# jcatalang/LUDVM

Hardware: AMD Instinct MI355X
Metric: biot_savart_pair_interactions_per_s (higher is better)
Workload: dtype f32

## Files before the change

ludvm_amd/csrc/pair_sym_kernels.hpp:

```cpp
#pragma once
#include <hip/hip_runtime.h>
#include "pair_kernels.hpp"
#include "sym_rule.hpp"

namespace ludvm {

struct SymScale {
  float scale;
  float pad;
  double inv;
};

struct SymArgs {
  const float* x; const float* z; const float* g;
  const float* xl; const float* zl;
  const float* cx; const float* cz;
  long long n;
  long long ntiles;
  long long dmax;
  long long i_first;
  long long i_count;
  int ysplit;
  int rsplit;
  int ytail;
  int rbulk;
  int xcd_run;
  long long tail_items;
  int diag_only;
  int tune_split, tune_rsplit;
  long long* acc_u; long long* acc_w;
  const SymScale* scale;
  long long* bad;
  float vc4;
  const long long* n_dev;
  int shard_rank, shard_world;
};

__device__ __forceinline__ unsigned long long fx_units(float v, float scale) {
  const float t = v * scale;
  const float a = __builtin_fabsf(t);
  const float h = __builtin_floorf(a * 2.3283064365386963e-10f);
  const float r = __builtin_fmaf(-h, 4294967296.0f, a);
  const unsigned long long m = ((unsigned long long)(unsigned)h << 32) | (unsigned long long)(unsigned)r;
  const unsigned long long s = (unsigned long long)((long long)__builtin_bit_cast(int, t) >> 31);
  return (m ^ s) - s;
}
__device__ __forceinline__ void fx_add(long long* acc, float v, float scale) {
  atomicAdd(reinterpret_cast<unsigned long long*>(acc), fx_units(v, scale));
}

__device__ __forceinline__ float dpp_rol1(float v) {
  const int i = __builtin_bit_cast(int, v);
  return __builtin_bit_cast(float, __builtin_amdgcn_update_dpp(i, i, 0x134, 0xf, 0xf, false));
}
__device__ __forceinline__ f32x2 dpp_rol1(f32x2 v) { return (f32x2){dpp_rol1(v.x), dpp_rol1(v.y)}; }

__device__ __forceinline__ f32x2 pk_sub_sel(f32x2 p, f32x2 s, int half) {
  f32x2 d;
  if (half) asm("v_pk_add_f32 %0, %1, %2 op_sel:[1,0] op_sel_hi:[1,1] neg_lo:[0,1] neg_hi:[0,1]" : "=v"(d) : "v"(p), "v"(s));
  else asm("v_pk_add_f32 %0, %1, %2 op_sel:[0,0] op_sel_hi:[0,1] neg_lo:[0,1] neg_hi:[0,1]" : "=v"(d) : "v"(p), "v"(s));
  return d;
}
__device__ __forceinline__ f32x2 pk_mul_sel(f32x2 s, f32x2 p, int half, f32x2 after) {
  f32x2 d;
  if (half) asm("v_pk_mul_f32 %0, %1, %2 op_sel:[0,1] op_sel_hi:[1,1]" : "=v"(d) : "v"(s), "v"(p), "v"(after));
  else asm("v_pk_mul_f32 %0, %1, %2 op_sel:[0,0] op_sel_hi:[1,0]" : "=v"(d) : "v"(s), "v"(p), "v"(after));
  return d;
}

__device__ __forceinline__ float load_or(const float* p, unsigned i, unsigned n, float pad) {
  const float v = p[i < n ? i : 0u];
  return i < n ? v : pad;
}

constexpr int kPlane = 96 * 4;
template <int T, int PLANE = kPlane>
__device__ __forceinline__ void slab_store(float* l, int home4, const float (&v)[T]) {
#pragma unroll
  for (int q = 0; q < T / 4; ++q) {
    const f32x4 V = (f32x4){v[4 * q], v[4 * q + 1], v[4 * q + 2], v[4 * q + 3]};
    *reinterpret_cast<f32x4*>(&l[q * PLANE + home4]) = V;
    if (PLANE > 256 && home4 < 128) *reinterpret_cast<f32x4*>(&l[q * PLANE + 256 + home4]) = V;
  }
}
template <int T, int PLANE = kPlane>
__device__ __forceinline__ void slab_load(const float* l, int home4, f32x2 (&out)[T / 2]) {
#pragma unroll
  for (int q = 0; q < T / 4; ++q) {
    const f32x4 V = *reinterpret_cast<const f32x4*>(&l[q * PLANE + home4]);
    out[2 * q] = (f32x2){V.x, V.y};
    out[2 * q + 1] = (f32x2){V.z, V.w};
  }
}

template <int T, bool HILO = false, int R = 1, bool RED = (R != 1)>
__global__ void __launch_bounds__(kBlock) __attribute__((amdgpu_waves_per_eu(T == 8 || HILO ? 3 : 4)))
pair_sym_f32(SymArgs a) {
  static_assert(T == 4 || T == 8, "T vortices per lane, read as T/4 ds_read_b128 per component");
  static_assert(R == 0 || R == 1 || R == 2 || R == 4, "waves per item");
  static_assert(RED == (R != 1), "one wave per item has nothing to reduce");
  constexpr int RR = R == 0 ? 4 : R;
  unsigned n = (unsigned)a.n, ntiles = (unsigned)a.ntiles, dmax = (unsigned)a.dmax, i_first = (unsigned)a.i_first,
           i_count = (unsigned)a.i_count;
  int ysplit = a.diag_only ? 1 : a.ysplit, ytail = a.ytail, rbulk = a.rbulk;
  if (a.n_dev) {
    n = (unsigned)*a.n_dev;
    unsigned dtot_;
    int rs_;
    sym_geometry_t<unsigned>(n, T, a.tune_split, R == 0 ? -1 : R, (unsigned)a.tail_items, ntiles, dmax, dtot_, ysplit, rs_, ytail,
                             rbulk);
    i_first = 0;
    i_count = ntiles;
    if (a.shard_world > 1) {
      unsigned long long f, cnt;
      shard_block(ntiles, a.shard_rank, a.shard_world, &f, &cnt);
      i_first = (unsigned)f;
      i_count = (unsigned)cnt;
    }
    if (a.diag_only) ysplit = 1;
  }
  constexpr int H = T / 2;
  constexpr int kWaves = kBlock / 64;
  constexpr int kComp = HILO ? 5 : 3;
  __shared__ __attribute__((aligned(16))) float slab[kWaves][kComp][(T / 4) * kPlane];
  static_assert(2 * T * 64 <= kComp * (T / 4) * kPlane, "partial sums fit the slab");
  __shared__ __attribute__((aligned(16))) float ioff[HILO ? 1 : kWaves][HILO ? 1 : 2][HILO ? 4 : 64 * T];

  const int lane = threadIdx.x & 63;
  const int wv = __builtin_amdgcn_readfirstlane((int)(threadIdx.x >> 6));
  const unsigned xcd = blockIdx.x % (unsigned)kXcds, qb = blockIdx.x / (unsigned)kXcds;
  unsigned yq = 0, unit = 0;
  bool active, shared;
  int rr = RR;
  if constexpr (R == 0) {
    const unsigned y1 = (unsigned)(ysplit - ytail);
    const unsigned rb = (unsigned)rbulk, ipb = (unsigned)kWaves / rb;
    const unsigned n_bulk = (unsigned)xcd_items(i_count, (unsigned)ysplit, xcd, 0, y1, a.xcd_run);
    const unsigned nb1 = (n_bulk * rb + 3) / 4;
    const bool tail = qb >= nb1;
    rr = tail ? 4 : (int)rb;
    shared = rr > 1;
    const unsigned q = tail ? qb - nb1 : qb * ipb + (unsigned)wv / rb;
    active = tail ? xcd_item(i_count, (unsigned)ysplit, xcd, y1, (unsigned)ytail, q, yq, unit, a.xcd_run)
                  : (q < n_bulk && xcd_item(i_count, (unsigned)ysplit, xcd, 0, y1, q, yq, unit, a.xcd_run));
    const bool wg_active = tail ? active : qb * ipb < n_bulk;
    if (!wg_active || (!shared && !active)) return;
  } else {
    shared = R > 1;
    const unsigned q = qb * (kWaves / R) + wv / R;
    active = xcd_item(i_count, (unsigned)ysplit, xcd, 0, (unsigned)ysplit, q, yq, unit, a.xcd_run);
  }
  const int r = shared ? wv % rr : 0;
  const int w0 = wv - r;
  if (R == 1 && !active) return;
  if (!active) { yq = 0; unit = 0; }
  const unsigned I = i_first + unit;
  const int y = (int)yq;
  const int ksteps = shared ? 64 / rr : 64;
  const int k_lo = r * ksteps;
  const int k_hi = k_lo + ksteps;
  constexpr unsigned W = 64u * T;
  float* const lx = slab[wv][0];
  float* const lz = slab[wv][1];
  float* const lg = slab[wv][2];
  float* const lxl = slab[wv][HILO ? 3 : 0];
  float* const lzl = slab[wv][HILO ? 4 : 1];

  const bool even = (ntiles % 2 == 0) && ntiles > 1;
  const int dtot = (int)dmax + (even ? 1 : 0);
  const int per = a.diag_only ? 0 : (int)(((unsigned)dtot + (unsigned)ysplit - 1) / (unsigned)ysplit);
  const int d_lo = 1 + y * per;
  int d_hi = d_lo + per;
  if (d_hi > dtot + 1) d_hi = dtot + 1;

  constexpr int NS = T / 4;
  f32x2 xp[H], zp[H], gp[H], au[T], aw[T], xpl[H], zpl[H];
  f32x2 xq[2][H], zq[2][H];
  {
    float x0[T], z0[T], g0[T], xl0[T], zl0[T];
#pragma unroll
    for (int t = 0; t < T; ++t) {
      const unsigned i = I * W + lane + 64u * t;
      const unsigned nl = active ? n : 0u;
      x0[t] = load_or(a.x, i, nl, kPadPosF); z0[t] = load_or(a.z, i, nl, kPadPosF); g0[t] = load_or(a.g, i, nl, 0.0f);
      xl0[t] = HILO ? load_or(a.xl, i, nl, 0.0f) : 0.0f; zl0[t] = HILO ? load_or(a.zl, i, nl, 0.0f) : 0.0f;
      au[t] = (f32x2){0.f, 0.f}; aw[t] = (f32x2){0.f, 0.f};
    }
#pragma unroll
    for (int h = 0; h < H; ++h) {
      xp[h] = (f32x2){x0[2 * h], x0[2 * h + 1]}; zp[h] = (f32x2){z0[2 * h], z0[2 * h + 1]};
      gp[h] = (f32x2){g0[2 * h], g0[2 * h + 1]};
      xpl[h] = (f32x2){xl0[2 * h], xl0[2 * h + 1]}; zpl[h] = (f32x2){zl0[2 * h], zl0[2 * h + 1]};
      xq[0][h] = xp[h]; xq[1][h] = xp[h]; zq[0][h] = zp[h]; zq[1][h] = zp[h];
    }
    if constexpr (!HILO) { slab_store<T, 256>(ioff[wv][0], lane * 4, x0); slab_store<T, 256>(ioff[wv][1], lane * 4, z0); }
  }
  const f32x2 vc4 = {a.vc4, a.vc4};
  const float fxs = a.scale->scale;
  const bool local = !HILO && a.cx != nullptr;
  const bool pl = (lane & 1) != 0;
  struct Org { float x0, x1, z0, z1; };
  auto scalar = [](float v) { return __builtin_bit_cast(float, __builtin_amdgcn_readfirstlane(__builtin_bit_cast(int, v))); };
  auto origin_records = [&](unsigned b) -> Org {
    const bool has = local && (b << kOriginShift) < n;
    const unsigned s0 = has ? 2 * b : 0;
    Org o{0.0f, 0.0f, 0.0f, 0.0f};
    if (has) { o.x0 = a.cx[s0]; o.x1 = a.cx[s0 + 1]; o.z0 = a.cz[s0]; o.z1 = a.cz[s0 + 1]; }
    return o;
  };
  auto to_scalars = [&](const Org& v) -> Org { return Org{scalar(v.x0), scalar(v.x1), scalar(v.z0), scalar(v.z1)}; };
  const unsigned blk_i = (I * W) >> kOriginShift;
  Org oi[NS];
#pragma unroll
  for (int q = 0; q < NS; ++q) oi[q] = to_scalars(origin_records(blk_i + q));
  float oix[NS], oiz[NS];
#pragma unroll
  for (int q = 0; q < NS; ++q) { oix[q] = pl ? oi[q].x1 : oi[q].x0; oiz[q] = pl ? oi[q].z1 : oi[q].z0; }
  auto refer_targets = [&](const Org oj) {
    f32x2 xo[H], zo[H];
    slab_load<T, 256>(ioff[HILO ? 0 : wv][0], lane * 4, xo);
    slab_load<T, 256>(ioff[HILO ? 0 : wv][HILO ? 0 : 1], lane * 4, zo);
#pragma unroll
    for (int rr = 0; rr < 2; ++rr) {
      const bool odd = pl != (rr != 0);
      const float jx = odd ? oj.x1 : oj.x0, jz = odd ? oj.z1 : oj.z0;
#pragma unroll
      for (int h = 0; h < H; ++h) {
        const float ddx = oix[h / 2] - jx, ddz = oiz[h / 2] - jz;
        xq[rr][h] = xo[h] + (f32x2){ddx, ddx};
        zq[rr][h] = zo[h] + (f32x2){ddz, ddz};
      }
    }
  };
  auto load_plane = [&](const float* l, int q, int pos4, f32x2 (&out)[2]) {
    const f32x4 V = *reinterpret_cast<const f32x4*>(&l[q * kPlane + pos4]);
    out[0] = (f32x2){V.x, V.y};
    out[1] = (f32x2){V.z, V.w};
  };
  float chk = 0.0f;
  const int lane32x4 = ((lane + 32) & 63) * 4;

  struct Round { unsigned J; bool diag, valid; };
  auto round_of = [&](int dd) -> Round {
    Round rd;
    rd.diag = dd < 0;
    const int d = rd.diag ? 0 : d_lo + dd;
    rd.valid = rd.diag || (active && dd < per && d < d_hi && !(even && d == dtot && I >= ntiles / 2));
    rd.J = I + (unsigned)d;
    if (rd.J >= ntiles) rd.J -= ntiles;
    return rd;
  };
  float pjx[T], pjz[T], pjg[T], pjxl[T], pjzl[T];
  Org poj[NS];
  auto fetch_tile = [&](const Round& rd) {
    const unsigned Jt = rd.valid ? rd.J : I;
    if ((Jt + 1) * W <= n) {
#pragma unroll
      for (int t = 0; t < T; ++t) {
        const unsigned j = Jt * W + lane + 64u * t;
        pjx[t] = a.x[j]; pjz[t] = a.z[j]; pjg[t] = a.g[j];
        pjxl[t] = HILO ? a.xl[j] : 0.0f; pjzl[t] = HILO ? a.zl[j] : 0.0f;
      }
    } else {
#pragma unroll
      for (int t = 0; t < T; ++t) {
        const unsigned j = Jt * W + lane + 64u * t;
        pjx[t] = load_or(a.x, j, n, kPadPosF); pjz[t] = load_or(a.z, j, n, kPadPosF); pjg[t] = load_or(a.g, j, n, 0.0f);
        pjxl[t] = HILO ? load_or(a.xl, j, n, 0.0f) : 0.0f; pjzl[t] = HILO ? load_or(a.zl, j, n, 0.0f) : 0.0f;
      }
    }
#pragma unroll
    for (int q = 0; q < NS; ++q) poj[q] = origin_records(((Jt * W) >> kOriginShift) + q);
  };
  constexpr bool kPrefetch = R != 0;
  const int dd0 = (active && y == 0) ? -1 : 0;
  if (kPrefetch) fetch_tile(round_of(dd0));
  for (int dd = dd0; dd < per; ++dd) {
    const Round rd = round_of(dd);
    if (!kPrefetch) fetch_tile(rd);
    const bool diag = rd.diag, valid = rd.valid;
    const unsigned J = rd.J;
    f32x2 bu[H], bw[H];
#pragma unroll
    for (int m = 0; m < H; ++m) { bu[m] = (f32x2){0.f, 0.f}; bw[m] = (f32x2){0.f, 0.f}; }
    Org oj[NS];
#pragma unroll
    for (int q = 0; q < NS; ++q) oj[q] = to_scalars(poj[q]);
    if (valid) {
      slab_store<T>(lx, lane * 4, pjx); slab_store<T>(lz, lane * 4, pjz); slab_store<T>(lg, lane * 4, pjg);
      if (HILO) { slab_store<T>(lxl, lane * 4, pjxl); slab_store<T>(lzl, lane * 4, pjzl); }
      __builtin_amdgcn_fence(__ATOMIC_RELEASE, "wavefront");
      __builtin_amdgcn_wave_barrier();
      __builtin_amdgcn_fence(__ATOMIC_ACQUIRE, "wavefront");
    }
    if (kPrefetch && dd + 1 < per) fetch_tile(round_of(dd + 1));
    if (valid) {

#pragma unroll
      for (int q = 0; q < NS; ++q) {
        if (local) refer_targets(oj[q]);
        for (int k = k_lo; k < k_hi; k += 2) {
          const int pos0 = ((k & 32) ? lane32x4 : lane * 4) + (k & 31) * 4;
#pragma unroll
          for (int rr = 0; rr < 2; ++rr) {
            const int pos = pos0 + 4 * rr;
            f32x2 xj[2], zj[2], gj[2], xjl[2], zjl[2];
            load_plane(lx, q, pos, xj); load_plane(lz, q, pos, zj); load_plane(lg, q, pos, gj);
            if (HILO) { load_plane(lxl, q, pos, xjl); load_plane(lzl, q, pos, zjl); }
#pragma unroll
            for (int mm = 0; mm < 2; ++mm) {
              const int m = 2 * q + mm;
#pragma unroll
              for (int t = 0; t < T; ++t) {
                f32x2 dx = pk_sub_sel(HILO ? xp[t / 2] : xq[rr][t / 2], xj[mm], t & 1);
                f32x2 dz = pk_sub_sel(HILO ? zp[t / 2] : zq[rr][t / 2], zj[mm], t & 1);
                if (HILO) { dx = dx + pk_sub_sel(xpl[t / 2], xjl[mm], t & 1); dz = dz + pk_sub_sel(zpl[t / 2], zjl[mm], t & 1); }
                f32x2 r2 = dx * dx;
                r2 = __builtin_elementwise_fma(dz, dz, r2);
                const f32x2 qq = __builtin_elementwise_fma(r2, r2, vc4);
                const f32x2 sv = {__builtin_amdgcn_rsqf(qq.x), __builtin_amdgcn_rsqf(qq.y)};
                const f32x2 sj = sv * gj[mm];
                const f32x2 si = pk_mul_sel(sv, gp[t / 2], t & 1, sj);
                au[t] = __builtin_elementwise_fma(dz, sj, au[t]);
                aw[t] = __builtin_elementwise_fma(dx, sj, aw[t]);
                bu[m] = __builtin_elementwise_fma(dz, si, bu[m]);
                bw[m] = __builtin_elementwise_fma(dx, si, bw[m]);
              }
            }
#pragma unroll
            for (int mm = 0; mm < 2; ++mm) { bu[2 * q + mm] = dpp_rol1(bu[2 * q + mm]); bw[2 * q + mm] = dpp_rol1(bw[2 * q + mm]); }
          }
        }
      }
      __builtin_amdgcn_fence(__ATOMIC_RELEASE, "wavefront");
      __builtin_amdgcn_wave_barrier();
    }
    const int home = (lane + k_hi) & 63;
    if (diag) continue;
    if (!RED || !shared) {
      if (valid) {
#pragma unroll
        for (int m = 0; m < H; ++m) {
          const unsigned j0 = J * W + home + 64u * (2 * m), j1 = j0 + 64;
          if (j0 < n) { fx_add(&a.acc_u[j0], -bu[m].x, fxs); fx_add(&a.acc_w[j0], -bw[m].x, fxs); }
          if (j1 < n) { fx_add(&a.acc_u[j1], -bu[m].y, fxs); fx_add(&a.acc_w[j1], -bw[m].y, fxs); }
        }
      }
    } else {
      if (valid) {
#pragma unroll
        for (int m = 0; m < H; ++m) {
          lx[(4 * m + 0) * 64 + home] = bu[m].x; lx[(4 * m + 1) * 64 + home] = bu[m].y;
          lx[(4 * m + 2) * 64 + home] = bw[m].x; lx[(4 * m + 3) * 64 + home] = bw[m].y;
        }
      }
      __syncthreads();
      if (valid) {
#pragma unroll 1
        for (int c = r; c < 2 * T; c += rr) {
          float v = 0.0f;
#pragma unroll
          for (int q = 0; q < RR; ++q)
            if (R != 0 || q < rr) v += (&slab[w0 + q][0][0])[c * 64 + lane];
          const unsigned j = J * W + lane + 64u * (2 * (c / 4) + (c & 1));
          if (j < n) fx_add((c & 2) ? &a.acc_w[j] : &a.acc_u[j], -v, fxs);
        }
      }
      __syncthreads();
    }
  }

  if (!RED || !shared) {
#pragma unroll
    for (int t = 0; t < T; ++t) {
      const unsigned i = I * W + lane + 64u * t;
      if (i < n) {
        const float su = au[t].x + au[t].y, sw = aw[t].x + aw[t].y;
        fx_add(&a.acc_u[i], su, fxs); fx_add(&a.acc_w[i], sw, fxs);
        chk += su + sw;
      }
    }
  } else {
#pragma unroll
    for (int t = 0; t < T; ++t) { lx[(2 * t) * 64 + lane] = au[t].x + au[t].y; lx[(2 * t + 1) * 64 + lane] = aw[t].x + aw[t].y; }
    __syncthreads();
    if (active) {
#pragma unroll 1
      for (int c = r; c < 2 * T; c += rr) {
        float v = 0.0f;
#pragma unroll
        for (int q = 0; q < RR; ++q)
          if (R != 0 || q < rr) v += (&slab[w0 + q][0][0])[c * 64 + lane];
        const unsigned i = I * W + lane + 64u * (c / 2);
        if (i < n) { fx_add((c & 1) ? &a.acc_w[i] : &a.acc_u[i], v, fxs); chk += v; }
      }
    }
  }
  if (!(__builtin_fabsf(chk) < __builtin_inff())) atomicAdd(reinterpret_cast<unsigned long long*>(a.bad), 1ULL);
}

template <int T>
__global__ void __launch_bounds__(kBlock) __attribute__((amdgpu_waves_per_eu(3)))
pair_sym_quad_f32(SymArgs a) {
  static_assert(T == 8, "the quad variant is built for the 512-vortex tile");
  constexpr int H = T / 2, NS = T / 4;
  constexpr unsigned W = 64u * T;
  constexpr int kWaves = kBlock / 64;
  static_assert(kWaves == (int)kQuad, "one I tile per wave");
  __shared__ __attribute__((aligned(16))) float slab[3][(T / 4) * kPlane];
  __shared__ __attribute__((aligned(16))) float ex[kWaves][2 * T * 64];
  __shared__ __attribute__((aligned(16))) float ioff[kWaves][2][64 * T];

  unsigned n = (unsigned)a.n, i_first = (unsigned)a.i_first, i_count = (unsigned)a.i_count;
  if (a.n_dev) {
    n = (unsigned)*a.n_dev;
    const unsigned nt = (n + W - 1) / W;
    i_first = 0;
    i_count = nt;
    if (a.shard_world > 1) {
      unsigned long long f, cnt;
      shard_block(nt, a.shard_rank, a.shard_world, &f, &cnt);
      i_first = (unsigned)f;
      i_count = (unsigned)cnt;
    }
  }
  const QuadGeom gm = quad_geometry<unsigned>(n, T, a.tune_split);
  const unsigned ntiles = gm.ntiles, dmax = gm.dmax;
  const int dtot = (int)gm.dtot;
  const bool even = (ntiles % 2 == 0) && ntiles > 1;

  const int lane = threadIdx.x & 63;
  const int wv = __builtin_amdgcn_readfirstlane((int)(threadIdx.x >> 6));
  const unsigned xcd = blockIdx.x % (unsigned)kXcds, qb = blockIdx.x / (unsigned)kXcds;
  const unsigned quads = (i_count + kQuad - 1) / kQuad;
  unsigned yq, quad;
  if (!xcd_item(quads, (unsigned)gm.ysplit, xcd, 0, (unsigned)gm.ysplit, qb, yq, quad, a.xcd_run)) return;
  const unsigned I0 = i_first + kQuad * quad;
  const unsigned I = I0 + (unsigned)wv;
  const bool mine = I < i_first + i_count && I < ntiles;
  int D_lo, D_hi;
  quad_chunk(gm, yq, D_lo, D_hi);
  const int per = D_hi - D_lo;

  float* const lx = slab[0];
  float* const lz = slab[1];
  float* const lg = slab[2];

  f32x2 gp[H], au[T], aw[T];
  f32x2 xq[2][H], zq[2][H];
  {
    float x0[T], z0[T], g0[T];
#pragma unroll
    for (int t = 0; t < T; ++t) {
      const unsigned i = I * W + lane + 64u * t;
      const unsigned nl = mine ? n : 0u;
      x0[t] = load_or(a.x, i, nl, kPadPosF); z0[t] = load_or(a.z, i, nl, kPadPosF); g0[t] = load_or(a.g, i, nl, 0.0f);
      au[t] = (f32x2){0.f, 0.f}; aw[t] = (f32x2){0.f, 0.f};
    }
#pragma unroll
    for (int h = 0; h < H; ++h) {
      gp[h] = (f32x2){g0[2 * h], g0[2 * h + 1]};
      xq[0][h] = (f32x2){x0[2 * h], x0[2 * h + 1]}; xq[1][h] = xq[0][h];
      zq[0][h] = (f32x2){z0[2 * h], z0[2 * h + 1]}; zq[1][h] = zq[0][h];
    }
    slab_store<T, 256>(ioff[wv][0], lane * 4, x0); slab_store<T, 256>(ioff[wv][1], lane * 4, z0);
  }
  const f32x2 vc4 = {a.vc4, a.vc4};
  const float fxs = a.scale->scale;
  const bool local = a.cx != nullptr;
  const bool pl = (lane & 1) != 0;
  struct Org { float x0, x1, z0, z1; };
  auto scalar = [](float v) { return __builtin_bit_cast(float, __builtin_amdgcn_readfirstlane(__builtin_bit_cast(int, v))); };
  auto origin_records = [&](unsigned b) -> Org {
    const bool has = local && (b << kOriginShift) < n;
    const unsigned s0 = has ? 2 * b : 0;
    Org o{0.0f, 0.0f, 0.0f, 0.0f};
    if (has) { o.x0 = a.cx[s0]; o.x1 = a.cx[s0 + 1]; o.z0 = a.cz[s0]; o.z1 = a.cz[s0 + 1]; }
    return o;
  };
  auto to_scalars = [&](const Org& v) -> Org { return Org{scalar(v.x0), scalar(v.x1), scalar(v.z0), scalar(v.z1)}; };
  float oix[NS], oiz[NS];
#pragma unroll
  for (int q = 0; q < NS; ++q) {
    const Org o = to_scalars(origin_records(mine ? ((I * W) >> kOriginShift) + q : 0xffffffffu >> kOriginShift));
    oix[q] = pl ? o.x1 : o.x0; oiz[q] = pl ? o.z1 : o.z0;
  }
  auto refer_targets = [&](const Org oj) {
    f32x2 xo[H], zo[H];
    slab_load<T, 256>(ioff[wv][0], lane * 4, xo);
    slab_load<T, 256>(ioff[wv][1], lane * 4, zo);
#pragma unroll
    for (int rr = 0; rr < 2; ++rr) {
      const bool odd = pl != (rr != 0);
      const float jx = odd ? oj.x1 : oj.x0, jz = odd ? oj.z1 : oj.z0;
#pragma unroll
      for (int h = 0; h < H; ++h) {
        const float ddx = oix[h / 2] - jx, ddz = oiz[h / 2] - jz;
        xq[rr][h] = xo[h] + (f32x2){ddx, ddx};
        zq[rr][h] = zo[h] + (f32x2){ddz, ddz};
      }
    }
  };
  auto load_plane = [&](const float* l, int q, int pos4, f32x2 (&out)[2]) {
    const f32x4 V = *reinterpret_cast<const f32x4*>(&l[q * kPlane + pos4]);
    out[0] = (f32x2){V.x, V.y};
    out[1] = (f32x2){V.z, V.w};
  };
  const int lane32x4 = ((lane + 32) & 63) * 4;
  float chk = 0.0f;

  const int qhome = 32 * (wv & 1) + (lane >> 1);
  float pjx[2], pjz[2], pjg[2];
  Org poj[NS];
  auto partner_of = [&](int dd) -> unsigned {
    unsigned J = I0 + (unsigned)(D_lo + dd);
    if (J >= ntiles) J -= ntiles;
    return J;
  };
  auto fetch_quarter = [&](int dd) {
    const unsigned J = (D_lo + dd < D_hi) ? partner_of(dd) : I0;
    const unsigned Jc = J < ntiles ? J : 0u;
#pragma unroll
    for (int s = 0; s < 2; ++s) {
      const unsigned j = Jc * W + (unsigned)qhome + 64u * (unsigned)(4 * (wv >> 1) + 2 * (lane & 1) + s);
      pjx[s] = load_or(a.x, j, n, kPadPosF); pjz[s] = load_or(a.z, j, n, kPadPosF); pjg[s] = load_or(a.g, j, n, 0.0f);
    }
#pragma unroll
    for (int q = 0; q < NS; ++q) poj[q] = origin_records(((Jc * W) >> kOriginShift) + q);
  };
  auto store_quarter = [&]() {
    const int at = (wv >> 1) * kPlane + 128 * (wv & 1) + 2 * lane;
    auto put = [&](float* l, const float (&v)[2]) {
      *reinterpret_cast<f32x2*>(&l[at]) = (f32x2){v[0], v[1]};
      if ((wv & 1) == 0) *reinterpret_cast<f32x2*>(&l[at + 256]) = (f32x2){v[0], v[1]};
    };
    put(lx, pjx); put(lz, pjz); put(lg, pjg);
  };

  fetch_quarter(0);
  for (int dd = 0; dd < per; ++dd) {
    const int D = D_lo + dd;
    if (D >= D_hi) break;
    const unsigned J = partner_of(dd);
    auto valid_of = [&](int w) -> bool {
      const int d = D - w;
      const unsigned Iw = I0 + (unsigned)w;
      const bool own = Iw < i_first + i_count && Iw < ntiles;
      return own && ((d >= 1 && d <= (int)dmax) || (even && d == dtot && Iw < ntiles / 2));
    };
    const bool valid = valid_of(wv);
    const bool any = valid_of(0) || valid_of(1) || valid_of(2) || valid_of(3);
    if (any) store_quarter();
    Org oj[NS];
#pragma unroll
    for (int q = 0; q < NS; ++q) oj[q] = to_scalars(poj[q]);
    __syncthreads();
    if (dd + 1 < per) fetch_quarter(dd + 1);
    if (!any) continue;
    f32x2 bu[H], bw[H];
#pragma unroll
    for (int m = 0; m < H; ++m) { bu[m] = (f32x2){0.f, 0.f}; bw[m] = (f32x2){0.f, 0.f}; }
    if (valid) {
#pragma unroll
      for (int q = 0; q < NS; ++q) {
        if (local) refer_targets(oj[q]);
        for (int k = 0; k < 64; k += 2) {
          const int pos0 = ((k & 32) ? lane32x4 : lane * 4) + (k & 31) * 4;
#pragma unroll
          for (int rr = 0; rr < 2; ++rr) {
            const int pos = pos0 + 4 * rr;
            f32x2 xj[2], zj[2], gj[2];
            load_plane(lx, q, pos, xj); load_plane(lz, q, pos, zj); load_plane(lg, q, pos, gj);
#pragma unroll
            for (int mm = 0; mm < 2; ++mm) {
              const int m = 2 * q + mm;
#pragma unroll
              for (int t = 0; t < T; ++t) {
                const f32x2 dx = pk_sub_sel(xq[rr][t / 2], xj[mm], t & 1);
                const f32x2 dz = pk_sub_sel(zq[rr][t / 2], zj[mm], t & 1);
                f32x2 r2 = dx * dx;
                r2 = __builtin_elementwise_fma(dz, dz, r2);
                const f32x2 qq = __builtin_elementwise_fma(r2, r2, vc4);
                const f32x2 sv = {__builtin_amdgcn_rsqf(qq.x), __builtin_amdgcn_rsqf(qq.y)};
                const f32x2 sj = sv * gj[mm];
                const f32x2 si = pk_mul_sel(sv, gp[t / 2], t & 1, sj);
                au[t] = __builtin_elementwise_fma(dz, sj, au[t]);
                aw[t] = __builtin_elementwise_fma(dx, sj, aw[t]);
                bu[m] = __builtin_elementwise_fma(dz, si, bu[m]);
                bw[m] = __builtin_elementwise_fma(dx, si, bw[m]);
              }
            }
#pragma unroll
            for (int mm = 0; mm < 2; ++mm) { bu[2 * q + mm] = dpp_rol1(bu[2 * q + mm]); bw[2 * q + mm] = dpp_rol1(bw[2 * q + mm]); }
          }
        }
      }
    }
#pragma unroll
    for (int m = 0; m < H; ++m) {
      ex[wv][(4 * m + 0) * 64 + lane] = bu[m].x; ex[wv][(4 * m + 1) * 64 + lane] = bu[m].y;
      ex[wv][(4 * m + 2) * 64 + lane] = bw[m].x; ex[wv][(4 * m + 3) * 64 + lane] = bw[m].y;
    }
    __syncthreads();
#pragma unroll 1
    for (int c = wv; c < 2 * T; c += kWaves) {
      float v = 0.0f;
#pragma unroll
      for (int w = 0; w < kWaves; ++w) v += ex[w][c * 64 + lane];
      const unsigned j = J * W + lane + 64u * (2 * (c / 4) + (c & 1));
      if (j < n) fx_add((c & 2) ? &a.acc_w[j] : &a.acc_u[j], -v, fxs);
    }
  }

  if (mine) {
#pragma unroll
    for (int t = 0; t < T; ++t) {
      const unsigned i = I * W + lane + 64u * t;
      if (i < n) {
        const float su = au[t].x + au[t].y, sw = aw[t].x + aw[t].y;
        fx_add(&a.acc_u[i], su, fxs); fx_add(&a.acc_w[i], sw, fxs);
        chk += su + sw;
      }
    }
  }
  if (!(__builtin_fabsf(chk) < __builtin_inff())) atomicAdd(reinterpret_cast<unsigned long long*>(a.bad), 1ULL);
}

constexpr int kPrepBlock = 1024;
__device__ __forceinline__ void sym_scale_from_sum(double sum_abs, double vc4, SymScale* out, long long* bad) {
  const double vc = sqrt(sqrt(vc4));
  const double bound = sum_abs / (1.4142135623730951 * vc);
  int e = 0;
  if (bound > 0.0 && bound < 1.0e300) (void)frexp(bound, &e);
  else if (!(bound == 0.0) && bad) atomicAdd(reinterpret_cast<unsigned long long*>(bad), 1ULL);
  int k = 61 - e;
  if (k > 120) k = 120;
  if (k < -120) k = -120;
  out->scale = (float)ldexp(1.0, k);
  out->pad = 0.0f;
  out->inv = ldexp(1.0, -k);
}

__device__ __forceinline__ double block_abs_sum(const float* g, long long first, long long count) {
  __shared__ double part[kPrepBlock / 64];
  double s[8] = {0, 0, 0, 0, 0, 0, 0, 0};
  const long long end = first + count;
  long long i = first + threadIdx.x;
  for (; i + 7 * kPrepBlock < end; i += 8 * kPrepBlock) {
#pragma unroll
    for (int k = 0; k < 8; ++k) s[k] += (double)__builtin_fabsf(g[i + k * kPrepBlock]);
  }
  for (int k = 0; i < end; i += kPrepBlock, ++k) s[k & 7] += (double)__builtin_fabsf(g[i]);
  double t = ((s[0] + s[1]) + (s[2] + s[3])) + ((s[4] + s[5]) + (s[6] + s[7]));
#pragma unroll
  for (int off = 32; off > 0; off >>= 1) t += __shfl_down(t, off, 64);
  __syncthreads();
  if ((threadIdx.x & 63) == 0) part[threadIdx.x >> 6] = t;
  __syncthreads();
  double tot = 0.0;
  for (int w = 0; w < (int)(blockDim.x >> 6); ++w) tot += part[w];
  return tot;
}

constexpr long long kPrepChunk = 65536;

__device__ __forceinline__ float fx_read(const long long* acc, long long i, const SymScale* sc, bool bad) {
  if (bad) return __builtin_nanf("");
  return (float)((double)acc[i] * sc->inv);
}
__device__ __forceinline__ float fx_read(const long long* acc, long long i, const SymScale* sc, const long long* bad) {
  return fx_read(acc, i, sc, *bad != 0);
}

constexpr int kFoilChunk = 256;
__device__ __forceinline__ void staged_sources_on(bool on, double xi, double zi, const double* x64, const double* z64,
                                                  const float* g32, long long first, int nsrc, float vc4, float& fu,
                                                  float& fw, int nextra = 0, const double* extra = nullptr) {
  __shared__ float fx[kFoilChunk], fz[kFoilChunk], fg[kFoilChunk];
  fu = 0.0f; fw = 0.0f;
  const int ntot = nsrc + nextra;
  if (ntot <= 0) return;
  const double ax = nsrc > 0 ? x64[first] : extra[0], az = nsrc > 0 ? z64[first] : extra[2];
  const float xr = (float)(xi - ax), zr = (float)(zi - az);
  for (int base = 0; base < ntot; base += kFoilChunk) {
    const int cnt = ntot - base < kFoilChunk ? ntot - base : kFoilChunk;
    __syncthreads();
    for (int t = threadIdx.x; t < cnt; t += blockDim.x) {
      const int q = base + t;
      if (q < nsrc) {
        fx[t] = (float)(x64[first + q] - ax);
        fz[t] = (float)(z64[first + q] - az);
        fg[t] = g32[first + q];
      } else {
        fx[t] = (float)(extra[q - nsrc] - ax);
        fz[t] = (float)(extra[2 + q - nsrc] - az);
        fg[t] = (float)extra[4 + q - nsrc];
      }
    }
    __syncthreads();
    if (on) {
      for (int j = 0; j < cnt; ++j) {
        const float dx = xr - fx[j], dz = zr - fz[j];
        const float r2 = __builtin_fmaf(dz, dz, dx * dx);
        const float k = fg[j] * __builtin_amdgcn_rsqf(__builtin_fmaf(r2, r2, vc4));
        fu = __builtin_fmaf(dz, k, fu);
        fw = __builtin_fmaf(dx, k, fw);
      }
    }
  }
}

}
```

Before: 9011 billion.

## Share one J-tile slab across the waves of an item via cooperative sliced loads

When several waves work on the same I tile, each wave now fetches only a slice of the J tile and writes it into a single shared slab owned by the item's first wave. Before, every wave loaded and stored the full tile into its own slab. Partial sums for the reductions move into separate regions of the slab memory, which removes the trailing syncthreads after the J-side reduction, and diagonal rounds are aligned across the workgroup so the barriers match. The change also adds a fast path for unmasked I-tile loads, replaces divisions with shifts, and uses clamped addressing for tail loads. In exchange it adds a block-wide barrier on every round, and the power-of-two shift assumptions on rr are fragile.

Result: no change. 8974 billion (-0.4%).

```diff
diff --git a/ludvm_amd/csrc/pair_sym_kernels.hpp b/ludvm_amd/csrc/pair_sym_kernels.hpp
--- a/ludvm_amd/csrc/pair_sym_kernels.hpp
+++ b/ludvm_amd/csrc/pair_sym_kernels.hpp
@@ -1,5 +1,6 @@
 #pragma once
 #include <hip/hip_runtime.h>
+#include <type_traits>
 #include "pair_kernels.hpp"
 #include "sym_rule.hpp"
 
@@ -123,7 +124,6 @@
   constexpr int kWaves = kBlock / 64;
   constexpr int kComp = HILO ? 5 : 3;
   __shared__ __attribute__((aligned(16))) float slab[kWaves][kComp][(T / 4) * kPlane];
-  static_assert(2 * T * 64 <= kComp * (T / 4) * kPlane, "partial sums fit the slab");
   __shared__ __attribute__((aligned(16))) float ioff[HILO ? 1 : kWaves][HILO ? 1 : 2][HILO ? 4 : 64 * T];
 
   const int lane = threadIdx.x & 63;
@@ -131,40 +131,59 @@
   const unsigned xcd = blockIdx.x % (unsigned)kXcds, qb = blockIdx.x / (unsigned)kXcds;
   unsigned yq = 0, unit = 0;
   bool active, shared;
+  bool other_diag = false;
   int rr = RR;
   if constexpr (R == 0) {
     const unsigned y1 = (unsigned)(ysplit - ytail);
-    const unsigned rb = (unsigned)rbulk, ipb = (unsigned)kWaves / rb;
+    const unsigned rb = (unsigned)rbulk, rsh = rb >> 1, ipb = (unsigned)kWaves >> rsh;
     const unsigned n_bulk = (unsigned)xcd_items(i_count, (unsigned)ysplit, xcd, 0, y1, a.xcd_run);
     const unsigned nb1 = (n_bulk * rb + 3) / 4;
     const bool tail = qb >= nb1;
     rr = tail ? 4 : (int)rb;
     shared = rr > 1;
-    const unsigned q = tail ? qb - nb1 : qb * ipb + (unsigned)wv / rb;
+    const unsigned q = tail ? qb - nb1 : qb * ipb + ((unsigned)wv >> rsh);
     active = tail ? xcd_item(i_count, (unsigned)ysplit, xcd, y1, (unsigned)ytail, q, yq, unit, a.xcd_run)
                   : (q < n_bulk && xcd_item(i_count, (unsigned)ysplit, xcd, 0, y1, q, yq, unit, a.xcd_run));
     const bool wg_active = tail ? active : qb * ipb < n_bulk;
     if (!wg_active || (!shared && !active)) return;
+    if (!tail && rb == 2) other_diag = (q ^ 1u) < n_bulk && (q ^ 1u) < xcd_share(i_count, xcd).n;
   } else {
     shared = R > 1;
     const unsigned q = qb * (kWaves / R) + wv / R;
     active = xcd_item(i_count, (unsigned)ysplit, xcd, 0, (unsigned)ysplit, q, yq, unit, a.xcd_run);
-  }
-  const int r = shared ? wv % rr : 0;
+    if (R == 2) other_diag = (q ^ 1u) < xcd_share(i_count, xcd).n;
+  }
+  const bool wg_diag = (active && yq == 0) || other_diag;
+  const int r = shared ? (wv & (rr - 1)) : 0;
   const int w0 = wv - r;
   if (R == 1 && !active) return;
   if (!active) { yq = 0; unit = 0; }
   const unsigned I = i_first + unit;
   const int y = (int)yq;
-  const int ksteps = shared ? 64 / rr : 64;
+  const int ksteps = shared ? (64 >> (rr >> 1)) : 64;
   const int k_lo = r * ksteps;
   const int k_hi = k_lo + ksteps;
   constexpr unsigned W = 64u * T;
-  float* const lx = slab[wv][0];
-  float* const lz = slab[wv][1];
-  float* const lg = slab[wv][2];
-  float* const lxl = slab[wv][HILO ? 3 : 0];
-  float* const lzl = slab[wv][HILO ? 4 : 1];
+  constexpr int kSlabF = kComp * (T / 4) * kPlane;
+  constexpr int kExF = 2 * T * 64;
+  constexpr int kFit = kSlabF / kExF;
+  static_assert(kFit >= 2 && kSlabF + 2 * kExF <= 2 * kSlabF, "two waves per item: slab and two sets of partial sums");
+  static_assert(kSlabF + (8 - kFit) * kExF <= 4 * kSlabF, "four waves per item: slab, four J-side and 4 - kFit I-side sets");
+  constexpr bool kMayShare = R != 1;
+  float* const ib = &slab[w0][0][0];
+  float* const lx = slab[w0][0];
+  float* const lz = slab[w0][1];
+  float* const lg = slab[w0][2];
+  float* const lxl = slab[w0][HILO ? 3 : 0];
+  float* const lzl = slab[w0][HILO ? 4 : 1];
+  float* const exw = ib + kSlabF + r * kExF;
+  auto is_off = [&](int q) -> int { return q < kFit ? q * kExF : kSlabF + (rr + q - kFit) * kExF; };
+  const int F = T >> (rr >> 1);
+  const int f0 = (r * 64 + lane) * F;
+  const int spl = f0 >> 8, swi = f0 & 255;
+  const unsigned sl_off = (unsigned)((swi >> 2) + 64 * (4 * spl + (swi & 3)));
+  const int sl_at = spl * kPlane + swi;
+  const bool sl_rep = swi < 128;
 
   const bool even = (ntiles % 2 == 0) && ntiles > 1;
   const int dtot = (int)dmax + (even ? 1 : 0);
@@ -178,14 +197,26 @@
   f32x2 xq[2][H], zq[2][H];
   {
     float x0[T], z0[T], g0[T], xl0[T], zl0[T];
-#pragma unroll
-    for (int t = 0; t < T; ++t) {
-      const unsigned i = I * W + lane + 64u * t;
-      const unsigned nl = active ? n : 0u;
-      x0[t] = load_or(a.x, i, nl, kPadPosF); z0[t] = load_or(a.z, i, nl, kPadPosF); g0[t] = load_or(a.g, i, nl, 0.0f);
-      xl0[t] = HILO ? load_or(a.xl, i, nl, 0.0f) : 0.0f; zl0[t] = HILO ? load_or(a.zl, i, nl, 0.0f) : 0.0f;
-      au[t] = (f32x2){0.f, 0.f}; aw[t] = (f32x2){0.f, 0.f};
-    }
+    if (active && (I + 1) * W <= n) {
+      const size_t i0 = (size_t)I * W;
+      const float *bx = a.x + i0, *bz = a.z + i0, *bg = a.g + i0, *bxl = HILO ? a.xl + i0 : nullptr, *bzl = HILO ? a.zl + i0 : nullptr;
+#pragma unroll
+      for (int t = 0; t < T; ++t) {
+        const unsigned o = (unsigned)lane + 64u * t;
+        x0[t] = bx[o]; z0[t] = bz[o]; g0[t] = bg[o];
+        xl0[t] = HILO ? bxl[o] : 0.0f; zl0[t] = HILO ? bzl[o] : 0.0f;
+      }
+    } else {
+#pragma unroll
+      for (int t = 0; t < T; ++t) {
+        const unsigned i = I * W + lane + 64u * t;
+        const unsigned nl = active ? n : 0u;
+        x0[t] = load_or(a.x, i, nl, kPadPosF); z0[t] = load_or(a.z, i, nl, kPadPosF); g0[t] = load_or(a.g, i, nl, 0.0f);
+        xl0[t] = HILO ? load_or(a.xl, i, nl, 0.0f) : 0.0f; zl0[t] = HILO ? load_or(a.zl, i, nl, 0.0f) : 0.0f;
+      }
+    }
+#pragma unroll
+    for (int t = 0; t < T; ++t) { au[t] = (f32x2){0.f, 0.f}; aw[t] = (f32x2){0.f, 0.f}; }
 #pragma unroll
     for (int h = 0; h < H; ++h) {
       xp[h] = (f32x2){x0[2 * h], x0[2 * h + 1]}; zp[h] = (f32x2){z0[2 * h], z0[2 * h + 1]};
@@ -245,39 +276,97 @@
     Round rd;
     rd.diag = dd < 0;
     const int d = rd.diag ? 0 : d_lo + dd;
-    rd.valid = rd.diag || (active && dd < per && d < d_hi && !(even && d == dtot && I >= ntiles / 2));
+    rd.valid = rd.diag ? (active && y == 0) : (active && dd < per && d < d_hi && !(even && d == dtot && I >= ntiles / 2));
     rd.J = I + (unsigned)d;
     if (rd.J >= ntiles) rd.J -= ntiles;
     return rd;
   };
-  float pjx[T], pjz[T], pjg[T], pjxl[T], pjzl[T];
+  constexpr int FN = R <= 1 ? T : T / R;
+  float pj[kComp][FN];
   Org poj[NS];
-  auto fetch_tile = [&](const Round& rd) {
-    const unsigned Jt = rd.valid ? rd.J : I;
+  const float* const src[5] = {a.x, a.z, a.g, a.xl, a.zl};
+  auto load_run = [&](auto cnt, const Round& rd, unsigned off0) {
+    constexpr int N = decltype(cnt)::value;
+    const unsigned Jv = rd.valid ? rd.J : I;
+    const unsigned Jt = Jv * W < n ? Jv : 0u;
+    const size_t j0 = (size_t)Jt * W;
+    unsigned ob = 4u * off0;
+    asm volatile("" : "+v"(ob));
     if ((Jt + 1) * W <= n) {
 #pragma unroll
-      for (int t = 0; t < T; ++t) {
-        const unsigned j = Jt * W + lane + 64u * t;
-        pjx[t] = a.x[j]; pjz[t] = a.z[j]; pjg[t] = a.g[j];
-        pjxl[t] = HILO ? a.xl[j] : 0.0f; pjzl[t] = HILO ? a.zl[j] : 0.0f;
+      for (int c = 0; c < kComp; ++c) {
+        const char* const b = reinterpret_cast<const char*>(src[c] + j0);
+#pragma unroll
+        for (int s = 0; s < N; ++s) pj[c][s] = *reinterpret_cast<const float*>(b + (size_t)ob + 256u * s);
       }
     } else {
-#pragma unroll
-      for (int t = 0; t < T; ++t) {
-        const unsigned j = Jt * W + lane + 64u * t;
-        pjx[t] = load_or(a.x, j, n, kPadPosF); pjz[t] = load_or(a.z, j, n, kPadPosF); pjg[t] = load_or(a.g, j, n, 0.0f);
-        pjxl[t] = HILO ? load_or(a.xl, j, n, 0.0f) : 0.0f; pjzl[t] = HILO ? load_or(a.zl, j, n, 0.0f) : 0.0f;
+      const unsigned last = 4u * (n - 1u - Jt * W);
+#pragma unroll
+      for (int c = 0; c < kComp; ++c) {
+        const char* const b = reinterpret_cast<const char*>(src[c] + j0);
+#pragma unroll
+        for (int s = 0; s < N; ++s) {
+          const unsigned o = ob + 256u * s;
+          const float v = *reinterpret_cast<const float*>(b + (size_t)(o < last ? o : last));
+          pj[c][s] = o <= last ? v : (c < 2 ? kPadPosF : 0.0f);
+        }
       }
     }
 #pragma unroll
     for (int q = 0; q < NS; ++q) poj[q] = origin_records(((Jt * W) >> kOriginShift) + q);
   };
-  constexpr bool kPrefetch = R != 0;
-  const int dd0 = (active && y == 0) ? -1 : 0;
-  if (kPrefetch) fetch_tile(round_of(dd0));
+  auto fetch_full = [&](const Round& rd) { load_run(std::integral_constant<int, R <= 1 ? T : 1>{}, rd, (unsigned)lane); };
+  auto store_full = [&]() {
+    if constexpr (R <= 1) {
+#pragma unroll
+      for (int c = 0; c < kComp; ++c) slab_store<T>(ib + c * (T / 4) * kPlane, lane * 4, pj[c]);
+    }
+  };
+  auto fetch_slice = [&](const Round& rd) {
+    if constexpr (R == 0) {
+      if (rr == 4) load_run(std::integral_constant<int, T / 4>{}, rd, sl_off);
+      else load_run(std::integral_constant<int, T / 2>{}, rd, sl_off);
+    } else {
+      load_run(std::integral_constant<int, T / RR>{}, rd, sl_off);
+    }
+  };
+  auto put_slice = [&](auto width) {
+    constexpr int FF = decltype(width)::value;
+#pragma unroll
+    for (int c = 0; c < kComp; ++c) {
+      float* const l = ib + c * (T / 4) * kPlane + sl_at;
+      if constexpr (FF == 1) {
+        *l = pj[c][0];
+        if (sl_rep) l[256] = pj[c][0];
+      } else {
+        typedef float vec_t __attribute__((ext_vector_type(FF)));
+        vec_t V;
+#pragma unroll
+        for (int s = 0; s < FF; ++s) V[s] = pj[c][s];
+        *reinterpret_cast<vec_t*>(l) = V;
+        if (sl_rep) *reinterpret_cast<vec_t*>(l + 256) = V;
+      }
+    }
+  };
+  auto store_slice = [&]() {
+    if constexpr (R == 0) {
+      if (rr == 4) put_slice(std::integral_constant<int, T / 4>{});
+      else put_slice(std::integral_constant<int, T / 2>{});
+    } else if constexpr (R > 1) {
+      put_slice(std::integral_constant<int, T / R>{});
+    }
+  };
+  (void)fetch_full; (void)store_full; (void)store_slice;
+  constexpr bool pf = R != 0 || !HILO;
+  const int dd0 = wg_diag ? -1 : 0;
+  auto fetch = [&](const Round& rd) {
+    if constexpr (R <= 1) { if (!(kMayShare && shared)) { fetch_full(rd); return; } }
+    fetch_slice(rd);
+  };
+  if (pf) fetch(round_of(dd0));
   for (int dd = dd0; dd < per; ++dd) {
     const Round rd = round_of(dd);
-    if (!kPrefetch) fetch_tile(rd);
+    if (!pf) fetch(rd);
     const bool diag = rd.diag, valid = rd.valid;
     const unsigned J = rd.J;
     f32x2 bu[H], bw[H];
@@ -286,14 +375,16 @@
     Org oj[NS];
 #pragma unroll
     for (int q = 0; q < NS; ++q) oj[q] = to_scalars(poj[q]);
-    if (valid) {
-      slab_store<T>(lx, lane * 4, pjx); slab_store<T>(lz, lane * 4, pjz); slab_store<T>(lg, lane * 4, pjg);
-      if (HILO) { slab_store<T>(lxl, lane * 4, pjxl); slab_store<T>(lzl, lane * 4, pjzl); }
+    if (kMayShare && shared) {
+      if (valid) store_slice();
+      __syncthreads();
+    } else if (valid) {
+      store_full();
       __builtin_amdgcn_fence(__ATOMIC_RELEASE, "wavefront");
       __builtin_amdgcn_wave_barrier();
       __builtin_amdgcn_fence(__ATOMIC_ACQUIRE, "wavefront");
     }
-    if (kPrefetch && dd + 1 < per) fetch_tile(round_of(dd + 1));
+    if (pf && dd + 1 < per) fetch(round_of(dd + 1));
     if (valid) {
 
 #pragma unroll
@@ -336,9 +427,8 @@
       __builtin_amdgcn_wave_barrier();
     }
     const int home = (lane + k_hi) & 63;
-    if (diag) continue;
     if (!RED || !shared) {
-      if (valid) {
+      if (valid && !diag) {
 #pragma unroll
         for (int m = 0; m < H; ++m) {
           const unsigned j0 = J * W + home + 64u * (2 * m), j1 = j0 + 64;
@@ -347,26 +437,27 @@
         }
       }
     } else {
-      if (valid) {
+      if (valid && !diag) {
 #pragma unroll
         for (int m = 0; m < H; ++m) {
-          lx[(4 * m + 0) * 64 + home] = bu[m].x; lx[(4 * m + 1) * 64 + home] = bu[m].y;
-          lx[(4 * m + 2) * 64 + home] = bw[m].x; lx[(4 * m + 3) * 64 + home] = bw[m].y;
+          exw[(4 * m + 0) * 64 + home] = bu[m].x; exw[(4 * m + 1) * 64 + home] = bu[m].y;
+          exw[(4 * m + 2) * 64 + home] = bw[m].x; exw[(4 * m + 3) * 64 + home] = bw[m].y;
         }
       }
       __syncthreads();
-      if (valid) {
+      if (valid && !diag) {
+        int ln = lane;
+        asm volatile("" : "+v"(ln));
 #pragma unroll 1
         for (int c = r; c < 2 * T; c += rr) {
           float v = 0.0f;
 #pragma unroll
           for (int q = 0; q < RR; ++q)
-            if (R != 0 || q < rr) v += (&slab[w0 + q][0][0])[c * 64 + lane];
+            if (R != 0 || q < rr) v += (ib + kSlabF + q * kExF)[c * 64 + ln];
           const unsigned j = J * W + lane + 64u * (2 * (c / 4) + (c & 1));
           if (j < n) fx_add((c & 2) ? &a.acc_w[j] : &a.acc_u[j], -v, fxs);
         }
       }
-      __syncthreads();
     }
   }
 
@@ -381,8 +472,9 @@
       }
     }
   } else {
-#pragma unroll
-    for (int t = 0; t < T; ++t) { lx[(2 * t) * 64 + lane] = au[t].x + au[t].y; lx[(2 * t + 1) * 64 + lane] = aw[t].x + aw[t].y; }
+    float* const isw = ib + is_off(r);
+#pragma unroll
+    for (int t = 0; t < T; ++t) { isw[(2 * t) * 64 + lane] = au[t].x + au[t].y; isw[(2 * t + 1) * 64 + lane] = aw[t].x + aw[t].y; }
     __syncthreads();
     if (active) {
 #pragma unroll 1
@@ -390,7 +482,7 @@
         float v = 0.0f;
 #pragma unroll
         for (int q = 0; q < RR; ++q)
-          if (R != 0 || q < rr) v += (&slab[w0 + q][0][0])[c * 64 + lane];
+          if (R != 0 || q < rr) v += (ib + is_off(q))[c * 64 + lane];
         const unsigned i = I * W + lane + 64u * (c / 2);
         if (i < n) { fx_add((c & 1) ? &a.acc_w[i] : &a.acc_u[i], v, fxs); chk += v; }
       }
```
